# redradman/MujocoPoseLearning

Hardware: AMD Instinct MI355X
Metric: env steps/sec (whole node), humanoid 'stand' task, 1/2/4/8 MI355X (higher is better)
Workload: dtype f64

## Files before the change

mujocoposelearning_amd/csrc/hs_contacts.h:

```cpp
#pragma once
#include "hs_lanes.h"
#include "hs_scratch.h"

namespace hs {
namespace {

template <typename T>
struct Con {
  T pos[3], n[3], t1[3], dist;
};

template <typename T>
__device__ __forceinline__ bool plane_sphere(const T* pp, const T* pn, const T* c, T r, Con<T>& o) {
  T d[3] = {c[0] - pp[0], c[1] - pp[1], c[2] - pp[2]};
  T cd = dot3(d, pn);
  if (cd > r) return false;
  o.dist = cd - r;
  for (int k = 0; k < 3; k++) { o.n[k] = pn[k]; o.pos[k] = c[k] - pn[k] * (o.dist * T(0.5) + r); o.t1[k] = 0; }
  return true;
}
template <typename T>
__device__ __forceinline__ bool sphere_sphere(const T* p1, T r1, const T* p2, T r2, Con<T>& o) {
  T d[3] = {p2[0] - p1[0], p2[1] - p1[1], p2[2] - p1[2]};
  T len = sqrt(dot3(d, d));
  T dist = len - r1 - r2;
  if (dist > 0) return false;
  o.dist = dist;
  if (len < T(1e-15)) { o.n[0] = 1; o.n[1] = 0; o.n[2] = 0; }
  else { T i = recip(len); for (int k = 0; k < 3; k++) o.n[k] = d[k] * i; }
  for (int k = 0; k < 3; k++) { o.pos[k] = p1[k] + o.n[k] * (r1 + dist * T(0.5)); o.t1[k] = 0; }
  return true;
}
template <typename T>
__device__ __forceinline__ void make_frame(Con<T>& c) {
  normalize3(c.n);
  if (sqrt(dot3(c.t1, c.t1)) < T(0.5)) {
    if (fabs(c.n[1]) < T(0.5)) { c.t1[0] = 0; c.t1[1] = 1; c.t1[2] = 0; }
    else { c.t1[0] = 0; c.t1[1] = 0; c.t1[2] = 1; }
  }
  T d = dot3(c.n, c.t1);
  for (int k = 0; k < 3; k++) c.t1[k] -= c.n[k] * d;
  normalize3(c.t1);
}

template <typename T, typename C>
__device__ __forceinline__ int collide_pair(const Scratch<T, C>& s, const int4 info, const T (&sz)[4], Con<T>& c0,
                                           Con<T>& c1) {
  const int g1 = info.x, g2 = info.y, fn = info.z;
  const T* p1 = s.u.k.gpos[g1];
  const T* p2 = s.u.k.gpos[g2];
  const T* a1 = s.u.k.gax[g1];
  const T* a2 = s.u.k.gax[g2];
  const T r1 = sz[0], h1 = sz[1], r2 = sz[2], h2 = sz[3];
  int n = 0;
  if (fn >= PAIR_SPHERE_SPHERE) {
    const T d[3] = {p1[0] - p2[0], p1[1] - p2[1], p1[2] - p2[2]};
    const T R = r1 + h1 + r2 + h2;
    if (dot3(d, d) > R * R) return 0;
  }
  if (fn == PAIR_PLANE_SPHERE) {
    n = plane_sphere(p1, a1, p2, r2, c0) ? 1 : 0;
  } else if (fn == PAIR_PLANE_CAPSULE) {
    T e[3];
    for (int k = 0; k < 3; k++) e[k] = p2[k] + h2 * a2[k];
    Con<T> t;
    if (plane_sphere(p1, a1, e, r2, t)) { for (int k = 0; k < 3; k++) t.t1[k] = a2[k]; c0 = t; n = 1; }
    for (int k = 0; k < 3; k++) e[k] = p2[k] - h2 * a2[k];
    if (plane_sphere(p1, a1, e, r2, t)) {
      for (int k = 0; k < 3; k++) t.t1[k] = a2[k];
      if (n == 0) c0 = t; else c1 = t;
      n++;
    }
  } else if (fn == PAIR_SPHERE_SPHERE) {
    n = sphere_sphere(p1, r1, p2, r2, c0) ? 1 : 0;
  } else if (fn == PAIR_SPHERE_CAPSULE) {
    T d[3] = {p1[0] - p2[0], p1[1] - p2[1], p1[2] - p2[2]};
    T x = dot3(a2, d);
    x = x > h2 ? h2 : (x < -h2 ? -h2 : x);
    T v[3] = {p2[0] + x * a2[0], p2[1] + x * a2[1], p2[2] + x * a2[2]};
    n = sphere_sphere(p1, r1, v, r2, c0) ? 1 : 0;
  } else {
    T ax1[3] = {a1[0] * h1, a1[1] * h1, a1[2] * h1}, ax2[3] = {a2[0] * h2, a2[1] * h2, a2[2] * h2};
    T dif[3] = {p1[0] - p2[0], p1[1] - p2[1], p1[2] - p2[2]};
    T ma = dot3(ax1, ax1), mb = -dot3(ax1, ax2), mc = dot3(ax2, ax2), u = -dot3(ax1, dif), v = dot3(ax2, dif);
    T det = ma * mc - mb * mb;
    T v1[3], v2[3];
    if (fabs(det) >= T(1e-15)) {
      T x1 = (mc * u - mb * v) / det, x2 = (ma * v - mb * u) / det;
      if (x1 > 1) { x1 = 1; x2 = (v - mb) / mc; }
      else if (x1 < -1) { x1 = -1; x2 = (v + mb) / mc; }
      if (x2 > 1) { x2 = 1; x1 = (u - mb) / ma; x1 = x1 > 1 ? 1 : (x1 < -1 ? -1 : x1); }
      else if (x2 < -1) { x2 = -1; x1 = (u + mb) / ma; x1 = x1 > 1 ? 1 : (x1 < -1 ? -1 : x1); }
      for (int k = 0; k < 3; k++) { v1[k] = p1[k] + x1 * ax1[k]; v2[k] = p2[k] + x2 * ax2[k]; }
      n = sphere_sphere(v1, r1, v2, r2, c0) ? 1 : 0;
    } else {
      for (int side = 1; side >= -1; side -= 2) {
        T x2 = (v - side * mb) / mc;
        x2 = x2 > 1 ? 1 : (x2 < -1 ? -1 : x2);
        for (int k = 0; k < 3; k++) { v1[k] = p1[k] + side * ax1[k]; v2[k] = p2[k] + x2 * ax2[k]; }
        Con<T> t;
        if (sphere_sphere(v1, r1, v2, r2, t)) { if (n == 0) c0 = t; else c1 = t; n++; }
      }
    }
  }
  if (n > 0) make_frame(c0);
  if (n > 1) make_frame(c1);
  return n;
}

template <typename T, typename C>
__device__ __forceinline__ void store_contact(MPtr<T> m, Scratch<T, C>& s, int slot, const Con<T>& c, int p) {
  if (slot >= C::CON) return;
  for (int k = 0; k < 3; k++) { s.con_pos[slot][k] = c.pos[k]; s.con_n[slot][k] = c.n[k]; s.con_t1[slot][k] = c.t1[k]; }
  s.con_dist[slot] = c.dist;
  s.con_pair[slot] = p;
  const int b1 = m->pair_b1[p], b2 = m->pair_b2[p];
  s.con_bb[slot] = (uint32_t)b1 | (uint32_t)b2 << 8 | (uint32_t)m->pair_dim[p] << 16;
  s.con_m1[slot] = b1 ? m->body_chainmask[b1] : 0u;
  s.con_m2[slot] = m->body_chainmask[b2];
  s.con_mu[slot] = m->pair_mu[p];
}

template <typename T>
__device__ __forceinline__ T impedance(CPtr<T> si, T pos, T margin) {
  T s0 = fmin(T(0.9999), fmax(T(0.0001), si[0])), s1 = fmin(T(0.9999), fmax(T(0.0001), si[1]));
  if (s0 == s1 || si[2] <= T(1e-15)) return T(0.5) * (s0 + s1);
  T x = (pos - margin) * si[5];
  if (x < 0) x = -x;
  if (x >= 1 || x <= 0) return x >= 1 ? s1 : s0;
  const T p = si[4];
  T y = x;
  if (p != T(1)) {
    const bool lo = x <= si[3];
    const T base = lo ? x : 1 - x;
    T pw = base * base;
    if (p != T(2)) pw = pow(base, p);
    y = lo ? pw * si[6] : 1 - pw * si[7];
  }
  return s0 + y * (s1 - s0);
}

template <typename T>
__device__ __forceinline__ uint32_t chain_mask(MPtr<T> m, int sl, int nb) {
  return (sl > 0 && sl < nb) ? m->body_chainmask[sl] : 0u;
}
template <int NV, typename T, typename C>
__device__ __forceinline__ void map_vx(Scratch<T, C>& s, int sl, int nb, uint32_t ch) {
  if (sl < nb) {
    T v[6] = {0, 0, 0, 0, 0, 0};
    for_bits<T>(ch, [&](int j) { ValsX<T, 6> r; r.x = s.vx[j]; for (int k = 0; k < 6; k++) r.v[k] = s.cdof[j][k]; return r; },
                [&](int, const ValsX<T, 6>& r) {
#pragma unroll
                  for (int k = 0; k < 6; k++) v[k] = fma(r.v[k], r.x, v[k]);
                });
    for (int k = 0; k < 6; k++) s.u.n.bvel[sl][k] = v[k];
  }
  WSYNC();
#pragma unroll
  for (int cs = 0; cs < C::CON; cs += HL) {
    const int c = cs + sl;
    if (c < s.ncon) {
      const uint32_t bb = s.con_bb[c];
      const int b1 = bb & 0xff, b2 = (bb >> 8) & 0xff;
      T r[3] = {s.con_pos[c][0] - s.com[0], s.con_pos[c][1] - s.com[1], s.con_pos[c][2] - s.com[2]};
      T w[3], v1[3], v2[3];
      cross3(s.u.n.bvel[b2], r, w);
      for (int k = 0; k < 3; k++) v2[k] = s.u.n.bvel[b2][3 + k] + w[k];
      cross3(s.u.n.bvel[b1], r, w);
      for (int k = 0; k < 3; k++) v1[k] = s.u.n.bvel[b1][3 + k] + w[k];
      T dv[3] = {v2[0] - v1[0], v2[1] - v1[1], v2[2] - v1[2]};
      T t2[3];
      cross3(s.con_n[c], s.con_t1[c], t2);
      s.con_v[c][0] = dot3(s.con_n[c], dv);
      s.con_v[c][1] = dot3(s.con_t1[c], dv);
      s.con_v[c][2] = dot3(t2, dv);
    }
  }
  WSYNC();
}

template <typename T, typename C>
__device__ __forceinline__ T row_Jx(MPtr<T> m, const Scratch<T, C>& s, int desc, T coef) {
  int kind = rk_kind(desc), j = rk_id(desc);
  if (kind <= RK_JHI) return coef * s.vx[j];
  if (kind <= RK_THI) {
    T v = 0;
    for (int w = 0; w < m->ten_nwrap[j]; w++) v += m->ten_wrapcoef[j][w] * s.vx[m->ten_wrapdof[j][w]];
    return coef * v;
  }
  int comp = kind == RK_CN ? 1 : 1 + ((kind - RK_P0) >> 1);
  return s.con_v[j][0] + coef * s.con_v[j][comp];
}

template <typename T, typename C>
__device__ __forceinline__ void row_u(MPtr<T> m, const Scratch<T, C>& s, int kind, int c, T* u) {
  if (kind == RK_CN) { for (int k = 0; k < 3; k++) u[k] = s.con_n[c][k]; return; }
  int sub = kind - RK_P0;
  T mu = s.con_mu[c];
  T sg = (sub & 1) ? -mu : mu;
  T t[3];
  if (sub >> 1) cross3(s.con_n[c], s.con_t1[c], t);
  else { t[0] = s.con_t1[c][0]; t[1] = s.con_t1[c][1]; t[2] = s.con_t1[c][2]; }
  for (int k = 0; k < 3; k++) u[k] = s.con_n[c][k] + sg * t[k];
}

template <typename T, typename C>
__device__ __forceinline__ void contact_aggregates(MPtr<T> m, Scratch<T, C>& s, int sl) {
  const bool up = threadIdx.x >= HL;
#pragma unroll
  for (int cs = 0; cs < C::CON; cs += HL) {
    const int c = cs + sl;
    bool act = false;
    if (c < s.ncon) {
      int adr = s.con_adr[c];
      int nr = (s.con_bb[c] >> 16) == 1 ? 1 : 4;
      T U[6] = {0, 0, 0, 0, 0, 0}, F[3] = {0, 0, 0};
      const bool pyr = nr == 4;
      T f4[4], D4[4], nn[3], t1[3], t2[3];
#pragma unroll
      for (int q = 0; q < 4; q++) {
        const bool on = q == 0 || pyr;
        f4[q] = on ? s.row_f[adr + q] : T(0);
        D4[q] = on ? s.row_D[adr + q] : T(0);
      }
      for (int k = 0; k < 3; k++) { nn[k] = s.con_n[c][k]; t1[k] = s.con_t1[c][k]; }
      const T mu = s.con_mu[c];
      cross3(nn, t1, t2);
#pragma unroll
      for (int q = 0; q < 4; q++) {
        const T f = f4[q];
        if (f != T(0)) {
          T u[3];
          if (!pyr) {
            for (int k = 0; k < 3; k++) u[k] = nn[k];
          } else {
            const T sg = (q & 1) ? -mu : mu;
            for (int k = 0; k < 3; k++) u[k] = nn[k] + sg * ((q >> 1) ? t2[k] : t1[k]);
          }
          const T D = D4[q];
          U[0] += D * u[0] * u[0]; U[1] += D * u[1] * u[1]; U[2] += D * u[2] * u[2];
          U[3] += D * u[0] * u[1]; U[4] += D * u[0] * u[2]; U[5] += D * u[1] * u[2];
          for (int k = 0; k < 3; k++) F[k] += f * u[k];
        }
      }
      for (int k = 0; k < 6; k++) s.con_U[c][k] = U[k];
      for (int k = 0; k < 3; k++) s.con_F[c][k] = F[k];
      act = F[0] != T(0) || F[1] != T(0) || F[2] != T(0) || U[0] != T(0) || U[1] != T(0) || U[2] != T(0);
    }
    const uint32_t mk = hballot(act, up);
    if (sl == 0) s.con_act[cs / HL] = mk;
  }
  WSYNC();
}
template <typename C, typename F>
__device__ __forceinline__ void for_active_contacts(const uint32_t* act, F&& f) {
#pragma unroll
  for (int w = 0; w < (C::CON + HL - 1) / HL; w++)
    for (uint32_t mk = act[w]; mk; mk &= mk - 1u) f(w * HL + __builtin_ctz(mk));
}

template <typename T, typename C, typename LD, typename F>
__device__ __forceinline__ void for_active_contacts_ld(const uint32_t* act, LD&& ld, F&& f) {
#pragma unroll
  for (int w = 0; w < (C::CON + HL - 1) / HL; w++)
    for_bits<T, true>(
        act[w], [&](int j) { return ld(w * HL + j); }, [&](int j, const auto& v) { f(w * HL + j, v); });
}

template <typename T, typename C>
__device__ __forceinline__ T jtf_lane(MPtr<T> m, const Scratch<T, C>& s, int sl, const T* cd) {
  T acc = 0;
  struct CV { uint32_t m1, m2; T p[3], f[3]; };
  for_active_contacts_ld<T, C>(s.con_act, [&](int c) {
    CV v;
    v.m1 = s.con_m1[c]; v.m2 = s.con_m2[c];
    for (int k = 0; k < 3; k++) { v.p[k] = s.con_pos[c][k]; v.f[k] = s.con_F[c][k]; }
    return v;
  }, [&](int, const CV& v) {
    const int in2 = bit(v.m2, sl), in1 = bit(v.m1, sl);
    if (in1 != in2) {
      T r[3] = {v.p[0] - s.com[0], v.p[1] - s.com[1], v.p[2] - s.com[2]};
      T w[3];
      cross3(cd, r, w);
      T jp[3] = {cd[3] + w[0], cd[4] + w[1], cd[5] + w[2]};
      T x = dot3(jp, v.f);
      acc += in2 ? x : -x;
    }
  });
  if (sl < MAXDOF) {
    int lr = s.lim_row[sl];
    int lo = (lr & 0xff) - 1, hi = (lr >> 8) - 1;
    if (lo >= 0) acc += s.row_f[lo];
    if (hi >= 0) acc -= s.row_f[hi];
  }
  for (int r = s.njl; r < s.nlim; r++) {
    int id = rk_id(s.row_kid[r]);
    T f = rk_kind(s.row_kid[r]) == RK_TLO ? s.row_f[r] : -s.row_f[r];
    for (int w = 0; w < m->ten_nwrap[id]; w++)
      if (m->ten_wrapdof[id][w] == sl) acc += f * m->ten_wrapcoef[id][w];
  }
  return acc;
}

}
}
```

mujocoposelearning_amd/csrc/hs_scratch.h:

```cpp
#pragma once
#include <cstdint>

#include "hs_lanes.h"
#include "hs_model.h"

namespace hs {
namespace {

enum RowKind { RK_JLO = 0, RK_JHI = 1, RK_TLO = 2, RK_THI = 3, RK_CN = 4, RK_P0 = 5 };
__device__ __forceinline__ int rk_kind(int kid) { return kid >> 16; }
__device__ __forceinline__ int rk_id(int kid) { return kid & 0xffff; }

template <typename T, typename C>
struct Scratch {
  T qpos[MAXQ];
  T qvel[MAXDOF];
  T ctrl[MAXU];
  alignas(16) T vx[MAXDOF];
  T com[4];
  T cinert[MAXBODY][10];
  T cdof[MAXDOF][6];
  T cvel[MAXBODY][6];
  T con_pos[C::CON][3];
  T con_n[C::CON][3];
  T con_t1[C::CON][3];
  T con_dist[C::CON];
  T con_v[C::CON][3];
  T con_U[C::CON][6];
  T con_F[C::CON][3];
  int con_pair[C::CON];
  int con_adr[C::CON];
  uint32_t con_bb[C::CON];
  uint32_t con_m1[C::CON];
  uint32_t con_m2[C::CON];
  T con_mu[C::CON];
  uint32_t con_act[(C::CON + HL - 1) / HL];
  uint16_t lim_row[MAXDOF];
  uint32_t dense_mask[C::RPL];
  int row_kid[C::EFC];
  T row_D[C::EFC];
  T row_f[C::EFC];
  int ncon, nefc, nlim, njl;
  int niter;
  struct Kin { T xpos[MAXBODY][3]; T xmat[MAXBODY][9]; T xquat[MAXBODY][4]; T xanchor[MAXJNT][3];
               T xaxis[MAXJNT][3]; T gpos[MAXGEOM][3]; T gax[MAXGEOM][3]; };
  union {
    Kin k;
    struct { T crb[MAXBODY][10]; T buf[MAXDOF][6]; } c;
    struct { T cdofdot[MAXDOF][6]; T cfrc[MAXBODY][6]; T csub[MAXBODY][6]; } r;
    struct { T bvel[MAXBODY][6];
             alignas(16) T cb[MAXDOF][2];
             T cfrc[MAXBODY][6], linv[MAXBODY][3], mv[MAXBODY][3]; } n;
    struct { alignas(16) float x[sizeof(T) == 8 ? 512 : 4]; alignas(16) float h[sizeof(T) == 8 ? 256 : 4]; } pol;
  } u;
};

constexpr int PGS_LA = 3;
template <typename T>
constexpr int pgs_cache_rows() { return sizeof(T) == 4 ? 40 : 48; }
template <typename T>
struct alignas(4 * sizeof(T)) PgsRow {
  T b, R, ar, ai;
  T g[4];
};
template <typename T, typename C>
struct PgsCache {
  static constexpr int NC = pgs_cache_rows<T>();
  T u[NC][MAXDOF];
  PgsRow<T> row[C::EFC];
};

}
}
```

mujocoposelearning_amd/csrc/hs_stepper.h:

```cpp
#pragma once
#include "hs_contacts.h"
#include "hs_dense.h"
#include "hs_lanes.h"
#include "hs_phase_clock.h"
#include "hs_scratch.h"

namespace hs {
namespace {

template <typename T, int NV, typename C>
struct Stepper {
  PhaseClock clk;
  MPtr<T> m;
  Scratch<T, C>& s;
  int sl, nb;
  bool up;
  T cd[6];
  T Mr[NV];
  T fsmooth;
  T fcon;
  T qacc;
  T qfa;
  T damp;
  int niter;
  T* dbg = nullptr;

  __device__ Stepper(MPtr<T> mm, Scratch<T, C>& ss, int lane)
      : m(mm), s(ss), sl(lane & (HL - 1)), nb(mm->nbody), up(lane >= HL) {}

  static constexpr bool LDLF = sizeof(T) == 8;
  static constexpr bool LDLE = false;
  __device__ __forceinline__ static KPtr<T> kargs() { return (KPtr<T>)__builtin_amdgcn_kernarg_segment_ptr(); }

  __device__ __forceinline__ void phase_begin() {
    m = opaque(m);
    sl = opaque_v(sl);
  }

  __device__ __forceinline__ void kinematics() {
    phase_begin();
    if (sl == 0) {
      for (int k = 0; k < 3; k++) s.u.k.xpos[0][k] = 0;
      s.u.k.xquat[0][0] = 1; s.u.k.xquat[0][1] = s.u.k.xquat[0][2] = s.u.k.xquat[0][3] = 0;
      for (int k = 0; k < 9; k++) s.u.k.xmat[0][k] = (k % 4 == 0) ? T(1) : T(0);
    }
    const int b = sl;
    const bool isb = b > 0 && b < nb;
    int depth = -1, par = 0, ja = 0, jn = 0, fqa = 0;
    bool isfree = false;
    T pl[3] = {0, 0, 0}, ql[4] = {1, 0, 0, 0};
    T anl[MAXJPB][3], axl[MAXJPB][3];
    if (isb) {
      depth = m->body_depth[b];
      par = m->body_parentid[b];
      ja = m->body_jntadr[b];
      jn = m->body_jntnum[b];
      isfree = jn == 1 && m->jnt_type[ja] == JNT_FREE;
      fqa = m->jnt_qposadr[ja];
      for (int k = 0; k < 3; k++) pl[k] = m->body_pos[b][k];
      for (int k = 0; k < 4; k++) ql[k] = m->body_quat[b][k];
    }
    if (isfree) {
      for (int k = 0; k < 3; k++) pl[k] = s.qpos[fqa + k];
      for (int k = 0; k < 4; k++) ql[k] = s.qpos[fqa + 3 + k];
    }
#pragma unroll
    for (int jj = 0; jj < MAXJPB; jj++) {
      const bool use = isb && !isfree && jj < jn;
      const int j = use ? ja + jj : 0;
      T jp[3], jx[3], ang = 0;
      for (int k = 0; k < 3; k++) { jp[k] = use ? m->jnt_pos[j][k] : T(0); jx[k] = use ? m->jnt_axis[j][k] : T(0); }
      if (use) {
        int qa = m->jnt_qposadr[j];
        ang = s.qpos[qa] - m->qpos0[qa];
      }
      T sn, cs;
      sincos_t(T(0.5) * ang, sn, cs);
      const T jr[4] = {cs, jx[0] * sn, jx[1] * sn, jx[2] * sn};
      T R[9];
      quat2mat(ql, R);
      mv3(R, jx, axl[jj]);
      mv3(R, jp, anl[jj]);
      for (int k = 0; k < 3; k++) anl[jj][k] += pl[k];
      if (use) {
        mulq(ql, jr, ql);
        quat2mat(ql, R);
        T v[3];
        mv3(R, jp, v);
        for (int k = 0; k < 3; k++) pl[k] = anl[jj][k] - v[k];
      }
    }
    WSYNC();
    for (int L = 1; L <= m->nlevel; L++) {
      if (depth == L) {
        T pos[3], q[4];
        if (isfree) {
          for (int k = 0; k < 3; k++) pos[k] = pl[k];
          for (int k = 0; k < 4; k++) q[k] = ql[k];
        } else {
          mv3(s.u.k.xmat[par], pl, pos);
          for (int k = 0; k < 3; k++) pos[k] += s.u.k.xpos[par][k];
          T pq[4] = {s.u.k.xquat[par][0], s.u.k.xquat[par][1], s.u.k.xquat[par][2], s.u.k.xquat[par][3]};
          mulq(pq, ql, q);
        }
        normalize4(q);
        for (int k = 0; k < 4; k++) s.u.k.xquat[b][k] = q[k];
        for (int k = 0; k < 3; k++) s.u.k.xpos[b][k] = pos[k];
        quat2mat(q, s.u.k.xmat[b]);
      }
      WSYNC();
    }
    if (isb) {
      if (isfree) {
        for (int k = 0; k < 3; k++) { s.u.k.xanchor[ja][k] = s.u.k.xpos[b][k]; s.u.k.xaxis[ja][k] = m->jnt_axis[ja][k]; }
      } else {
        const T* Rp = s.u.k.xmat[par];
        const T* xp = s.u.k.xpos[par];
#pragma unroll
        for (int jj = 0; jj < MAXJPB; jj++) {
          if (jj < jn) {
            T an[3], ax[3];
            mv3(Rp, anl[jj], an);
            mv3(Rp, axl[jj], ax);
            for (int k = 0; k < 3; k++) { s.u.k.xanchor[ja + jj][k] = xp[k] + an[k]; s.u.k.xaxis[ja + jj][k] = ax[k]; }
          }
        }
      }
    }
    if (sl < m->ngeom) {
      int g = sl, gb = m->geom_bodyid[g];
      T gp[3] = {m->geom_pos[g][0], m->geom_pos[g][1], m->geom_pos[g][2]};
      T gz[3] = {m->geom_zaxis[g][0], m->geom_zaxis[g][1], m->geom_zaxis[g][2]};
      T w[3];
      mv3(s.u.k.xmat[gb], gp, w);
      for (int k = 0; k < 3; k++) s.u.k.gpos[g][k] = s.u.k.xpos[gb][k] + w[k];
      mv3(s.u.k.xmat[gb], gz, s.u.k.gax[g]);
    }
    T mx = 0, my = 0, mz = 0, xi[3] = {0, 0, 0};
    if (b > 0 && b < nb) {
      T ip[3] = {m->body_ipos[b][0], m->body_ipos[b][1], m->body_ipos[b][2]}, w[3];
      mv3(s.u.k.xmat[b], ip, w);
      for (int k = 0; k < 3; k++) xi[k] = s.u.k.xpos[b][k] + w[k];
      T mb = m->body_mass[b];
      mx = mb * xi[0]; my = mb * xi[1]; mz = mb * xi[2];
    }
    T inv = T(1) / m->total_mass;
    T c0 = hsum(mx) * inv, c1 = hsum(my) * inv, c2 = hsum(mz) * inv;
    if (sl == 0) { s.com[0] = c0; s.com[1] = c1; s.com[2] = c2; }
    if (b > 0 && b < nb) {
      const T* R = s.u.k.xmat[b];
      CPtr<T> I6 = m->body_inert[b];
      T I[9] = {I6[0], I6[3], I6[4], I6[3], I6[1], I6[5], I6[4], I6[5], I6[2]};
      T A[9];
      for (int r = 0; r < 3; r++)
        for (int c = 0; c < 3; c++) A[3 * r + c] = R[3 * r] * I[c] + R[3 * r + 1] * I[3 + c] + R[3 * r + 2] * I[6 + c];
      T Ic[6];
      Ic[0] = A[0] * R[0] + A[1] * R[1] + A[2] * R[2];
      Ic[1] = A[3] * R[3] + A[4] * R[4] + A[5] * R[5];
      Ic[2] = A[6] * R[6] + A[7] * R[7] + A[8] * R[8];
      Ic[3] = A[0] * R[3] + A[1] * R[4] + A[2] * R[5];
      Ic[4] = A[0] * R[6] + A[1] * R[7] + A[2] * R[8];
      Ic[5] = A[3] * R[6] + A[4] * R[7] + A[5] * R[8];
      T d[3] = {xi[0] - c0, xi[1] - c1, xi[2] - c2};
      T mass = m->body_mass[b];
      T* ci = s.cinert[b];
      ci[0] = Ic[0] + mass * (d[1] * d[1] + d[2] * d[2]);
      ci[1] = Ic[1] + mass * (d[0] * d[0] + d[2] * d[2]);
      ci[2] = Ic[2] + mass * (d[0] * d[0] + d[1] * d[1]);
      ci[3] = Ic[3] - mass * d[0] * d[1];
      ci[4] = Ic[4] - mass * d[0] * d[2];
      ci[5] = Ic[5] - mass * d[1] * d[2];
      ci[6] = mass * d[0]; ci[7] = mass * d[1]; ci[8] = mass * d[2]; ci[9] = mass;
    }
    if (sl == 0)
      for (int k = 0; k < 10; k++) s.cinert[0][k] = 0;
    for (int k = 0; k < 6; k++) cd[k] = 0;
    if (sl < NV) {
      int j = m->dof_jntid[sl], db = m->dof_bodyid[sl];
      T off[3] = {c0 - s.u.k.xanchor[j][0], c1 - s.u.k.xanchor[j][1], c2 - s.u.k.xanchor[j][2]};
      T ax[3];
      bool lin = false;
      if (m->jnt_type[j] == JNT_FREE) {
        int k = sl - m->jnt_dofadr[j];
        if (k < 3) {
          lin = true;
          cd[3] = k == 0 ? T(1) : T(0); cd[4] = k == 1 ? T(1) : T(0); cd[5] = k == 2 ? T(1) : T(0);
        } else {
          int c = k - 3;
          ax[0] = s.u.k.xmat[db][c]; ax[1] = s.u.k.xmat[db][3 + c]; ax[2] = s.u.k.xmat[db][6 + c];
        }
      } else {
        ax[0] = s.u.k.xaxis[j][0]; ax[1] = s.u.k.xaxis[j][1]; ax[2] = s.u.k.xaxis[j][2];
      }
      if (!lin) {
        cd[0] = ax[0]; cd[1] = ax[1]; cd[2] = ax[2];
        cross3(ax, off, cd + 3);
      }
      for (int k = 0; k < 6; k++) s.cdof[sl][k] = cd[k];
    }
    WSYNC();
    if (dbg)
      for (int k = sl; k < MAXBODY * 3; k += HL) dbg[k] = s.u.k.xpos[k / 3][k % 3];
  }

  __device__ __forceinline__ int collision() {
    phase_begin();
    int ncon = 0;
    const int npair = m->npair;
    int4 info_n = make_int4(0, 0, 0, 0);
    T sz_n[4] = {0, 0, 0, 0};
    if (sl < npair) {
      info_n = make_int4(m->pair_info[sl][0], m->pair_info[sl][1], m->pair_info[sl][2], m->pair_info[sl][3]);
      for (int k = 0; k < 4; k++) sz_n[k] = m->pair_size[sl][k];
    }
    for (int base = 0; base < npair; base += HL) {
      int p = base + sl;
      Con<T> c0, c1;
      int n = 0;
      const int4 info = info_n;
      T sz[4] = {sz_n[0], sz_n[1], sz_n[2], sz_n[3]};
      if (p + HL < npair) {
        info_n = make_int4(m->pair_info[p + HL][0], m->pair_info[p + HL][1], m->pair_info[p + HL][2],
                           m->pair_info[p + HL][3]);
        for (int k = 0; k < 4; k++) sz_n[k] = m->pair_size[p + HL][k];
      }
      if (p < npair) n = collide_pair(s, info, sz, c0, c1);
      uint32_t m1 = hballot(n >= 1, up), m2 = hballot(n >= 2, up);
      int pre = below(m1, sl) + below(m2, sl);
      if (n >= 1) store_contact(m, s, ncon + pre, c0, p);
      if (n >= 2) store_contact(m, s, ncon + pre + 1, c1, p);
      ncon += __popc(m1) + __popc(m2);
    }
    int overflow = ncon > C::CON;
    if (overflow) ncon = C::CON;
    if (sl == 0) s.ncon = ncon;
    WSYNC();
    return overflow;
  }

  __device__ __forceinline__ void mass_matrix() {
    phase_begin();
    if (sl > 0 && sl < nb) {
      const uint32_t dm = m->body_descmask[sl] & ~1u & ((nb < 32 ? (1u << nb) : 0u) - 1u);
      T a[10] = {0, 0, 0, 0, 0, 0, 0, 0, 0, 0};
      for_bits<T>(dm, [&](int c) { Vals<T, 10> r; for (int k = 0; k < 10; k++) r.v[k] = s.cinert[c][k]; return r; },
                  [&](int, const Vals<T, 10>& r) { for (int k = 0; k < 10; k++) a[k] += r.v[k]; });
      for (int k = 0; k < 10; k++) s.u.c.crb[sl][k] = a[k];
    }
    WSYNC();
    T bf[6] = {0, 0, 0, 0, 0, 0};
    uint32_t anci = 0;
    T arm = 0;
    if (sl < NV) {
      mul_inert(s.u.c.crb[m->dof_bodyid[sl]], cd, bf);
      for (int k = 0; k < 6; k++) s.u.c.buf[sl][k] = bf[k];
      anci = m->dof_ancmask[sl];
      arm = m->dof_armature[sl];
    }
    WSYNC();
    {
      T cb2[2][12];
      auto load = [&](auto jc, T (&dst)[12]) {
        constexpr int j = decltype(jc)::value;
        for (int k = 0; k < 6; k++) { dst[k] = s.cdof[j][k]; dst[6 + k] = s.u.c.buf[j][k]; }
      };
      load(std::integral_constant<int, 0>{}, cb2[0]);
      static_for<0, NV>([&](auto jc) {
        constexpr int j = decltype(jc)::value;
        if constexpr (j + 1 < NV) load(std::integral_constant<int, j + 1>{}, cb2[(j + 1) & 1]);
        SCHED_FENCE();
        const uint32_t ancj = m->dof_ancmask[j];
        const bool rel = (sl < NV) && (bit(anci, j) || bit(ancj, sl));
        const T* cj = cb2[j & 1];
        const T v = (j <= sl) ? dot6(cj, bf) : dot6(cd, cj + 6);
        Mr[j] = rel ? v + ((j == sl) ? arm : T(0)) : T(0);
      });
    }
    WSYNC();
  }

  __device__ __forceinline__ void velocity_forces() {
    phase_begin();
    if (sl < nb) {
      T v[6] = {0, 0, 0, 0, 0, 0};
      if (sl > 0) {
        const uint32_t ch = m->body_chainmask[sl];
        for_bits<T>(ch, [&](int j) { ValsX<T, 6> r; r.x = s.qvel[j]; for (int k = 0; k < 6; k++) r.v[k] = s.cdof[j][k]; return r; },
                    [&](int, const ValsX<T, 6>& r) { for (int k = 0; k < 6; k++) v[k] = fma(r.v[k], r.x, v[k]); });
      }
      for (int k = 0; k < 6; k++) s.cvel[sl][k] = v[k];
    }
    if (sl < NV) {
      const uint32_t dm = m->dof_dotmask[sl];
      T v[6] = {0, 0, 0, 0, 0, 0}, cdd[6];
      for_bits<T>(dm, [&](int j) { ValsX<T, 6> r; r.x = s.qvel[j]; for (int k = 0; k < 6; k++) r.v[k] = s.cdof[j][k]; return r; },
                  [&](int, const ValsX<T, 6>& r) { for (int k = 0; k < 6; k++) v[k] = fma(r.v[k], r.x, v[k]); });
      cross_motion(v, cd, cdd);
      for (int k = 0; k < 6; k++) s.u.r.cdofdot[sl][k] = cdd[k];
    }
    WSYNC();
    if (sl > 0 && sl < nb) {
      const uint32_t ch = m->body_chainmask[sl];
      T a[6] = {0, 0, 0, -m->gravity[0], -m->gravity[1], -m->gravity[2]};
      for_bits<T>(ch, [&](int j) { ValsX<T, 6> r; r.x = s.qvel[j]; for (int k = 0; k < 6; k++) r.v[k] = s.u.r.cdofdot[j][k]; return r; },
                  [&](int, const ValsX<T, 6>& r) { for (int k = 0; k < 6; k++) a[k] = fma(r.v[k], r.x, a[k]); });
      T f[6], t[6], t2[6];
      mul_inert(s.cinert[sl], a, f);
      mul_inert(s.cinert[sl], s.cvel[sl], t);
      cross_force(s.cvel[sl], t, t2);
      for (int k = 0; k < 6; k++) s.u.r.cfrc[sl][k] = f[k] + t2[k];
    }
    WSYNC();
    if (sl > 0 && sl < nb) {
      const uint32_t dm = m->body_descmask[sl] & ~1u & ((nb < 32 ? (1u << nb) : 0u) - 1u);
      T a[6] = {0, 0, 0, 0, 0, 0};
      for_bits<T>(dm, [&](int c) { Vals<T, 6> r; for (int k = 0; k < 6; k++) r.v[k] = s.u.r.cfrc[c][k]; return r; },
                  [&](int, const Vals<T, 6>& r) { for (int k = 0; k < 6; k++) a[k] += r.v[k]; });
      for (int k = 0; k < 6; k++) s.u.r.csub[sl][k] = a[k];
    }
    WSYNC();
    fsmooth = 0;
    qfa = 0;
    if (sl < NV) {
      T bias = dot6(cd, s.u.r.csub[m->dof_bodyid[sl]]);
      int qa = m->dof_qposadr[sl];
      T pas = -m->dof_damping[sl] * s.qvel[sl];
      if (qa >= 0) pas -= m->dof_stiffness[sl] * (s.qpos[qa] - m->dof_springref[sl]);
      int u = m->dof_actuator[sl];
      if (u >= 0) {
        T c = s.ctrl[u];
        if (m->act_ctrllimited[u]) c = fmin(m->act_ctrlrange[u][1], fmax(m->act_ctrlrange[u][0], c));
        qfa = m->act_gear[u] * c;
      }
      fsmooth = pas - bias + qfa;
    }
    WSYNC();
  }

  __device__ __forceinline__ int rows(T (&D)[C::RPL], T (&ar)[C::RPL], int (&rd)[C::RPL], T (&rc)[C::RPL]) {
    phase_begin();
    damp = sl < NV ? m->dof_damping[sl] : T(0);
    int overflow = 0;
    int ncon = s.ncon;
    int nrow = 0;
    {
      bool lo = false, hi = false;
      if (sl < m->njnt && m->jnt_limited[sl]) {
        T q = s.qpos[m->jnt_qposadr[sl]];
        lo = (q - m->jnt_range[sl][0]) < m->jnt_margin[sl];
        hi = (m->jnt_range[sl][1] - q) < m->jnt_margin[sl];
      }
      uint32_t ml = hballot(lo, up), mh = hballot(hi, up);
      int pre = below(ml, sl) + below(mh, sl);
      if (lo) s.row_kid[pre] = (RK_JLO << 16) | sl;
      if (hi) s.row_kid[pre + lo] = (RK_JHI << 16) | sl;
      nrow = __popc(ml) + __popc(mh);
      s.lim_row[sl] = 0;
      if (lo || hi)
        s.lim_row[m->jnt_dofadr[sl]] = (uint16_t)((lo ? pre + 1 : 0) | (hi ? (pre + lo + 1) << 8 : 0));
    }
    const int njl = nrow;
    {
      bool lo = false, hi = false;
      if (sl < m->ntendon && m->ten_limited[sl]) {
        T L = 0;
        for (int w = 0; w < m->ten_nwrap[sl]; w++) L += m->ten_wrapcoef[sl][w] * s.qpos[m->ten_wrapqadr[sl][w]];
        lo = (L - m->ten_range[sl][0]) < m->ten_margin[sl];
        hi = (m->ten_range[sl][1] - L) < m->ten_margin[sl];
      }
      uint32_t ml = hballot(lo, up), mh = hballot(hi, up);
      int pre = nrow + below(ml, sl) + below(mh, sl);
      if (lo) s.row_kid[pre] = (RK_TLO << 16) | sl;
      if (hi) s.row_kid[pre + lo] = (RK_THI << 16) | sl;
      nrow += __popc(ml) + __popc(mh);
    }
    int nlim = nrow;
    {
      int tot = 0;
#pragma unroll
      for (int cs = 0; cs < C::CON; cs += HL) {
        const int c = cs + sl;
        const bool isc = c < ncon;
        const bool pyr = isc && (s.con_bb[c] >> 16) == 3;
        tot += __popc(hballot(isc, up)) + 3 * __popc(hballot(pyr, up));
      }
      if (nrow + tot > C::EFC) {
        overflow = 1;
        int fit = 0, nr = nrow;
        for (int c = 0; c < ncon; c++) {
          int need = (s.con_bb[c] >> 16) == 3 ? 4 : 1;
          if (nr + need > C::EFC) break;
          nr += need;
          fit++;
        }
        ncon = fit;
      }
#pragma unroll
      for (int cs = 0; cs < C::CON; cs += HL) {
        const int c = cs + sl;
        const bool isc = c < ncon;
        const bool pyr = isc && (s.con_bb[c] >> 16) == 3;
        const uint32_t mc = hballot(isc, up), mp = hballot(pyr, up);
        const int pre = nrow + below(mc, sl) + 3 * below(mp, sl);
        if (isc) {
          s.con_adr[c] = pre;
          if (!pyr) s.row_kid[pre] = (RK_CN << 16) | c;
          else for (int q = 0; q < 4; q++) s.row_kid[pre + q] = ((RK_P0 + q) << 16) | c;
        }
        nrow += __popc(mc) + 3 * __popc(mp);
      }
    }
    if (sl == 0) { s.ncon = ncon; s.nefc = nrow; s.nlim = nlim; s.njl = njl; }
    if (sl < NV) s.vx[sl] = s.qvel[sl];
    WSYNC();
    map_vx<NV>(s, sl, nb, chain_mask(m, sl, nb));
#pragma unroll
    for (int q = 0; q < C::RPL; q++) {
      int r = sl + HL * q;
      D[q] = 0;
      ar[q] = 0;
      rd[q] = 0;
      rc[q] = 0;
      bool dense = false;
      if (r < nrow) {
        int kid = s.row_kid[r];
        int kind = rk_kind(kid), id = rk_id(kid);
        T pos, margin, dA, rscale = 1;
        CPtr<T> sr;
        CPtr<T> si;
        if (kind <= RK_JHI) {
          T qv = s.qpos[m->jnt_qposadr[id]];
          pos = kind == RK_JLO ? qv - m->jnt_range[id][0] : m->jnt_range[id][1] - qv;
          margin = m->jnt_margin[id];
          sr = m->jnt_solref[id]; si = m->jnt_solimp[id];
          int dof = m->jnt_dofadr[id];
          dA = m->dof_invweight0[dof];
          rd[q] = (kind << 16) | dof;
          rc[q] = kind == RK_JLO ? T(1) : T(-1);
        } else if (kind <= RK_THI) {
          T L = 0;
          for (int w = 0; w < m->ten_nwrap[id]; w++) L += m->ten_wrapcoef[id][w] * s.qpos[m->ten_wrapqadr[id][w]];
          pos = kind == RK_TLO ? L - m->ten_range[id][0] : m->ten_range[id][1] - L;
          margin = m->ten_margin[id];
          sr = m->ten_solref[id]; si = m->ten_solimp[id];
          dA = m->ten_invweight0[id];
          rd[q] = kid;
          rc[q] = kind == RK_TLO ? T(1) : T(-1);
          dense = true;
        } else {
          int p = s.con_pair[id];
          pos = s.con_dist[id];
          margin = m->pair_margin[p];
          sr = m->pair_solref[p]; si = m->pair_solimp[p];
          const uint32_t bb = s.con_bb[id];
          T tran = m->body_invweight_tran[bb & 0xff] + m->body_invweight_tran[(bb >> 8) & 0xff];
          T mu = s.con_mu[id];
          dA = kind == RK_CN ? tran : tran + mu * mu * tran;
          if (kind != RK_CN) rscale = 2 * mu * mu;
          rd[q] = kid;
          rc[q] = kind == RK_CN ? T(0) : (((kind - RK_P0) & 1) ? -mu : mu);
          dense = s.con_m1[id] != 0u;
        }
        T imp = impedance(si, pos, margin);
        T dmax = fmin(T(0.9999), fmax(T(0.0001), si[1]));
        T K, B;
        if (sr[0] > 0) {
          T tc = fmax(sr[0], 2 * m->timestep), dr = sr[1];
          const T u = recip(dmax * tc), ud = u * recip(dr);
          K = ud * ud;
          B = 2 * u;
        } else {
          const T v = recip(dmax);
          K = -sr[0] * v * v;
          B = -sr[1] * v;
        }
        T R = rscale * fmax(T(1e-15), (1 - imp) * dA * recip(imp));
        D[q] = recip(R);
        s.row_D[r] = D[q];
        ar[q] = -B * row_Jx(m, s, rd[q], rc[q]) - K * imp * (pos - margin);
      }
      uint32_t dm = hballot(dense, up);
      if (sl == 0) s.dense_mask[q] = dm;
    }
    WSYNC();
    return overflow;
  }

  __device__ __forceinline__ void solve(T xws, int maxit, T tol, const T (&D)[C::RPL], const T (&ar)[C::RPL],
                                        const int (&rd)[C::RPL], const T (&rc)[C::RPL]) {
    phase_begin();
    const int nefc = s.nefc;
    T x = sl < NV ? xws : T(0);
    bool vr[C::RPL];
#pragma unroll
    for (int q = 0; q < C::RPL; q++) vr[q] = sl + HL * q < nefc;
    const uint32_t anci = sl < NV ? m->dof_ancmask[sl] : 0u;
    const uint32_t bch = chain_mask(m, sl, nb);
    const T scale = m->newton_scale;
    if (sl < NV) s.vx[sl] = x;
    WSYNC();
    T Mx = matvec_lds(Mr, s.vx);
    map_vx<NV>(s, sl, nb, bch);
    T jar[C::RPL], Js[C::RPL];
#pragma unroll
    for (int q = 0; q < C::RPL; q++) jar[q] = vr[q] ? row_Jx(m, s, rd[q], rc[q]) - ar[q] : T(0);
    HS_STAMP(clk, 6);
    bool done = false;
    int it = 0;
    if (sl == 0) s.niter = maxit;
    for (; it < maxit; it++) {
      m = opaque(m);
      sl = opaque_v(sl);
      bool act[C::RPL];
#pragma unroll
      for (int q = 0; q < C::RPL; q++) {
        act[q] = vr[q] && jar[q] < 0;
        if (vr[q]) s.row_f[sl + HL * q] = act[q] ? -D[q] * jar[q] : T(0);
      }
      WSYNC();
      contact_aggregates(m, s, sl);
      HS_STAMP(clk, 7);
      T jtf = jtf_lane(m, s, sl, cd);
      T g = sl < NV ? Mx - fsmooth - jtf : T(0);
      const T gn2 = hsum(g * g);
      const bool conv = scale * scale * gn2 < tol * tol;
      if (conv && !done && sl == 0) s.niter = it;
      done = done || conv;
      HS_STAMP(clk, 8);
      if (__ballot(!done) == 0) break;
      T H[NV];
      T hdinv = 0, hdiag = 0;
      {
        T aug[6] = {0, 0, 0, 0, 0, 0};
        T dadd = 0;
        struct CU { uint32_t m1, m2; T p[3], U[6]; };
        for_active_contacts_ld<T, C>(s.con_act, [&](int c) {
          CU v;
          v.m1 = s.con_m1[c]; v.m2 = s.con_m2[c];
          for (int k = 0; k < 3; k++) v.p[k] = s.con_pos[c][k];
          for (int k = 0; k < 6; k++) v.U[k] = s.con_U[c][k];
          return v;
        }, [&](int, const CU& v) {
          if (v.m1 != 0u || !bit(v.m2, sl)) return;
          T r[3] = {v.p[0] - s.com[0], v.p[1] - s.com[1], v.p[2] - s.com[2]};
          T w[3];
          cross3(cd, r, w);
          T jp[3] = {cd[3] + w[0], cd[4] + w[1], cd[5] + w[2]};
          const T* U = v.U;
          T z[3] = {U[0] * jp[0] + U[3] * jp[1] + U[4] * jp[2], U[3] * jp[0] + U[1] * jp[1] + U[5] * jp[2],
                    U[4] * jp[0] + U[5] * jp[1] + U[2] * jp[2]};
          T rz[3];
          cross3(r, z, rz);
          for (int k = 0; k < 3; k++) { aug[k] += rz[k]; aug[3 + k] += z[k]; }
        });
        {
          int lr = s.lim_row[sl];
          int lo = (lr & 0xff) - 1, hi = (lr >> 8) - 1;
          if (lo >= 0 && s.row_f[lo] != T(0)) dadd += s.row_D[lo];
          if (hi >= 0 && s.row_f[hi] != T(0)) dadd += s.row_D[hi];
        }
        HS_STAMP(clk, 27);
        constexpr int HESS_G = sizeof(T) == 8 ? 2 : 1;
        if constexpr (HESS_G == 1) {
#pragma unroll
          for (int j = 0; j < NV; j++) {
            T cj[6];
            for (int k = 0; k < 6; k++) cj[k] = s.cdof[j][k];
            H[j] = Mr[j] + (bit(anci, j) ? dot6(cj, aug) : T(0)) + ((j == sl) ? dadd : T(0));
            SCHED_FENCE();
          }
        } else {
          constexpr int NG = (NV + HESS_G - 1) / HESS_G;
          T cbuf[2][HESS_G][6];
          auto load = [&](auto gc, T (&dst)[HESS_G][6]) {
            constexpr int j0 = decltype(gc)::value * HESS_G;
            static_for<0, HESS_G>([&](auto tc) {
              constexpr int t = decltype(tc)::value;
              if constexpr (j0 + t < NV)
                for (int k = 0; k < 6; k++) dst[t][k] = s.cdof[j0 + t][k];
            });
          };
          load(std::integral_constant<int, 0>{}, cbuf[0]);
          static_for<0, NG>([&](auto gc) {
            constexpr int g = decltype(gc)::value, j0 = g * HESS_G;
            if constexpr (g + 1 < NG) load(std::integral_constant<int, g + 1>{}, cbuf[(g + 1) & 1]);
            SCHED_FENCE();
            static_for<0, HESS_G>([&](auto tc) {
              constexpr int t = decltype(tc)::value, j = j0 + t;
              if constexpr (j < NV)
                H[j] = Mr[j] + (bit(anci, j) ? dot6(cbuf[g & 1][t], aug) : T(0)) + ((j == sl) ? dadd : T(0));
            });
          });
        }
        HS_STAMP(clk, 28);
        uint32_t dm[C::RPL];
#pragma unroll
        for (int q = 0; q < C::RPL; q++) dm[q] = s.dense_mask[q] & hballot(act[q], up);
        for (;;) {
          int r = -1;
#pragma unroll
          for (int q = C::RPL - 1; q >= 0; q--)
            if (dm[q]) r = HL * q + __builtin_ctz(dm[q]);
          if (__ballot(r >= 0) == 0) break;
          T jr = 0, Dr = 0;
          if (r >= 0) {
            dm[r / HL] &= dm[r / HL] - 1u;
            if (s.row_f[r] != T(0)) {
              int kid = s.row_kid[r];
              int kind = rk_kind(kid), id = rk_id(kid);
              Dr = s.row_D[r];
              if (kind == RK_TLO || kind == RK_THI) {
                for (int w = 0; w < m->ten_nwrap[id]; w++)
                  if (m->ten_wrapdof[id][w] == sl) jr += m->ten_wrapcoef[id][w];
                if (kind == RK_THI) jr = -jr;
              } else {
                int in2 = bit(s.con_m2[id], sl), in1 = bit(s.con_m1[id], sl);
                if (in1 != in2) {
                  T rr[3] = {s.con_pos[id][0] - s.com[0], s.con_pos[id][1] - s.com[1], s.con_pos[id][2] - s.com[2]};
                  T w[3], u[3];
                  cross3(cd, rr, w);
                  T jp[3] = {cd[3] + w[0], cd[4] + w[1], cd[5] + w[2]};
                  row_u(m, s, kind, id, u);
                  jr = in2 ? dot3(u, jp) : -dot3(u, jp);
                }
              }
            }
          }
          if (sl >= NV) jr = 0;
          T dj = Dr * jr;
          static_for<0, NV>([&](auto jc) {
            constexpr int j = decltype(jc)::value;
            H[j] += dj * bcast<j>(jr);
          });
        }
      }
      HS_STAMP(clk, 9);
      chol_rows<NV, T, LDLF>(H, hdinv, sl, s.u.n.cb, &hdiag);
      HS_STAMP(clk, 15);
      T sdir = -chol_solve<NV, T, LDLF>(H, hdinv, g, sl);
      if (sl >= NV) sdir = 0;
      HS_STAMP(clk, 10);
      if (sl < NV) s.vx[sl] = sdir;
      WSYNC();
      T Ms = matvec_lds(Mr, s.vx);
      T A0 = hsum(sl < NV ? sdir * Ms : T(0));
      T B0 = hsum(sl < NV ? sdir * (Mx - fsmooth) : T(0));
      HS_STAMP(clk, 18);
      map_vx<NV>(s, sl, nb, bch);
      HS_STAMP(clk, 19);
#pragma unroll
      for (int q = 0; q < C::RPL; q++) Js[q] = vr[q] ? row_Jx(m, s, rd[q], rc[q]) : T(0);
      HS_STAMP(clk, 16);
      bool same1 = true;
#pragma unroll
      for (int q = 0; q < C::RPL; q++) same1 = same1 && (!vr[q] || ((jar[q] + Js[q] < 0) == act[q]));
      bool lsdone = done || (hballot(!same1, up) == 0);
      T alpha = 1, lo = 0, hi = T(1e30);
      T d0 = 0;
      {
        T c = 0;
#pragma unroll
        for (int q = 0; q < C::RPL; q++) c += act[q] ? D[q] * jar[q] * Js[q] : T(0);
        d0 = B0 + hsum(c);
      }
      const T ltol = (sizeof(T) == 8 ? T(1e-10) : T(1e-5)) * fabs(d0);
      for (int ls = 0; ls < 30; ls++) {
        if (__ballot(!lsdone) == 0) break;
        T c1 = 0, c2 = 0;
#pragma unroll
        for (int q = 0; q < C::RPL; q++) {
          T jq = jar[q] + alpha * Js[q];
          bool a = vr[q] && jq < 0;
          c1 += a ? D[q] * jq * Js[q] : T(0);
          c2 += a ? D[q] * Js[q] * Js[q] : T(0);
        }
        T d1 = B0 + alpha * A0 + hsum(c1);
        T d2 = A0 + hsum(c2);
        if (!lsdone) {
          if (fabs(d1) <= ltol) {
            lsdone = true;
          } else {
            if (d1 < 0) lo = alpha; else hi = alpha;
            T an = d2 > 0 ? alpha - d1 * recip(d2) : T(-1);
            if (!(an > lo && an < hi)) an = hi < T(1e29) ? T(0.5) * (lo + hi) : T(2) * alpha;
            if (hi - lo <= (sizeof(T) == 8 ? T(1e-14) : T(1e-6)) * hi) lsdone = true;
            else alpha = an;
          }
        }
      }
      HS_STAMP(clk, 11);
      if (!done) {
        x += alpha * sdir;
        Mx += alpha * Ms;
        bool changed = false;
#pragma unroll
        for (int q = 0; q < C::RPL; q++) {
          T nj = jar[q] + alpha * Js[q];
          changed = changed || (vr[q] && ((nj < 0) != act[q]));
          jar[q] = nj;
        }
        if (hballot(changed, up) == 0 && fabs(alpha - T(1)) < T(1e-3)) {
          done = true;
          if (sl == 0) s.niter = it + 1;
        }
      }
      if (__ballot(!done) == 0) { it++; break; }
    }
    WSYNC();
    niter = s.niter;
#pragma unroll
    for (int q = 0; q < C::RPL; q++)
      if (vr[q]) s.row_f[sl + HL * q] = jar[q] < 0 ? -D[q] * jar[q] : T(0);
    WSYNC();
    contact_aggregates(m, s, sl);
    fcon = sl < NV ? jtf_lane(m, s, sl, cd) : T(0);
    qacc = x;
    WSYNC();
    HS_STAMP(clk, 12);
  }

  __device__ __forceinline__ T row_J_lane(int r) {
    if (sl >= NV) return T(0);
    const int kid = s.row_kid[r];
    const int kind = rk_kind(kid), id = rk_id(kid);
    if (kind <= RK_JHI) return m->jnt_dofadr[id] == sl ? (kind == RK_JLO ? T(1) : T(-1)) : T(0);
    if (kind <= RK_THI) {
      T v = 0;
      for (int w = 0; w < m->ten_nwrap[id]; w++)
        if (m->ten_wrapdof[id][w] == sl) v += m->ten_wrapcoef[id][w];
      return kind == RK_TLO ? v : -v;
    }
    const int in2 = bit(s.con_m2[id], sl), in1 = bit(s.con_m1[id], sl);
    if (in1 == in2) return T(0);
    T rr[3] = {s.con_pos[id][0] - s.com[0], s.con_pos[id][1] - s.com[1], s.con_pos[id][2] - s.com[2]};
    T w[3], u[3];
    cross3(cd, rr, w);
    T jp[3] = {cd[3] + w[0], cd[4] + w[1], cd[5] + w[2]};
    row_u(m, s, kind, id, u);
    const T v = dot3(u, jp);
    return in2 ? v : -v;
  }

  __device__ __forceinline__ void solve_pgs(T xws, int maxit, const T (&D)[C::RPL], const T (&ar)[C::RPL],
                                            const int (&rd)[C::RPL], const T (&rc)[C::RPL], PgsCache<T, C>& pc) {
    phase_begin();
    const int nefc = s.nefc;
    const uint32_t bch = chain_mask(m, sl, nb);
    const T fs = sl < NV ? fsmooth : T(0);
    constexpr int NC = PgsCache<T, C>::NC;
    constexpr int LA = PGS_LA;
    bool vr[C::RPL];
#pragma unroll
    for (int q = 0; q < C::RPL; q++) vr[q] = sl + HL * q < nefc;
    T L[NV];
#pragma unroll
    for (int j = 0; j < NV; j++) L[j] = Mr[j];
    T dinv = 0;
    chol_rows<NV>(L, dinv, sl, s.u.n.cb);
    if (sl < NV) s.vx[sl] = xws;
    WSYNC();
    map_vx<NV>(s, sl, nb, bch);
    T wc = 0;
#pragma unroll
    for (int q = 0; q < C::RPL; q++) {
      const int r = sl + HL * q;
      if (vr[q]) {
        const T jar = row_Jx(m, s, rd[q], rc[q]) - ar[q];
        const T f = jar < 0 ? -D[q] * jar : T(0);
        const T R = recip(D[q]);
        s.row_f[r] = f;
        pc.row[r].b = -ar[q];
        pc.row[r].R = R;
        wc += f * (T(0.5) * R * f - ar[q]);
      }
    }
    WSYNC();
    int maxr = nefc;
    maxr = max(maxr, __shfl_xor(maxr, HL));
    constexpr int G = sizeof(T) == 8 ? 4 : 8;
    const int ncache = maxr < NC ? maxr : NC;
    for (int r0 = 0; r0 < ncache; r0 += G) {
      T y[G];
      static_for<0, G>([&](auto gc) {
        constexpr int g = decltype(gc)::value;
        y[g] = r0 + g < nefc ? row_J_lane(r0 + g) : T(0);
      });
      chol_fwd_multi<NV, G>(L, dinv, y, sl);
      static_for<0, G>([&](auto gc) {
        constexpr int g = decltype(gc)::value;
        if (r0 + g < NC) pc.u[r0 + g][sl] = sl < NV ? y[g] : T(0);
      });
    }
    WSYNC();
    auto urow = [&](int r) -> T {
      if (r < NC) return pc.u[r][sl];
      T y = chol_fwd<NV>(L, dinv, r < nefc ? row_J_lane(r) : T(0), sl);
      return sl < NV ? y : T(0);
    };
    {
      T uw[LA + 1];
#pragma unroll
      for (int j = 0; j < LA; j++) uw[j] = 0;
      for (int r = 0; r < maxr; r++) {
        uw[LA] = urow(r);
        const T a = hsum(uw[LA] * uw[LA]);
        T gr[LA];
#pragma unroll
        for (int j = 1; j <= LA; j++) gr[j - 1] = hsum(uw[LA] * uw[LA - j]);
        if (r < nefc && sl == 0) {
          const T arr = a + pc.row[r].R;
          pc.row[r].ar = arr;
          pc.row[r].ai = recip(arr < T(1e-15) ? T(1e-15) : arr);
#pragma unroll
          for (int j = 0; j < LA; j++) pc.row[r].g[j] = gr[j];
        }
#pragma unroll
        for (int j = 0; j < LA; j++) uw[j] = uw[j + 1];
      }
    }
    WSYNC();
    contact_aggregates(m, s, sl);
    T z, y0;
    {
      T y2[2] = {fs, fs + (sl < NV ? jtf_lane(m, s, sl, cd) : T(0))};
      chol_fwd_multi<NV, 2>(L, dinv, y2, sl);
      y0 = sl < NV ? y2[0] : T(0);
      z = sl < NV ? y2[1] : T(0);
    }
    if (hsum(wc + T(0.5) * (z * z - y0 * y0)) > T(0)) {
#pragma unroll
      for (int q = 0; q < C::RPL; q++)
        if (vr[q]) s.row_f[sl + HL * q] = 0;
      z = y0;
    }
    WSYNC();
    const T scale = m->newton_scale, tol = m->pgs_tol;
    bool done = false;
    int it = 0;
    for (int sweep = 0; sweep < maxit; sweep++) {
      m = opaque(m);
      sl = opaque_v(sl);
      T improvement = 0;
      auto sweep_rows = [&](auto fastc) {
        constexpr bool FAST = decltype(fastc)::value;
        auto uget = [&](int r) -> T {
          if constexpr (FAST) return pc.u[r][sl];
          else return urow(r);
        };
        constexpr int RING = LA + 1;
        static_assert(RING % 2 == 0, "P/F double buffer alternates with the row parity");
        T U[RING], S[RING], Dl[RING];
#pragma unroll
        for (int i = 0; i < RING; i++) {
          U[i] = (i < LA && i < maxr) ? uget(i) : T(0);
          S[i] = i < LA ? hsum(U[i] * z) : T(0);
          Dl[i] = 0;
        }
        PgsRow<T> P[2];
        T F[2];
        P[0] = pc.row[0];
        F[0] = nefc > 0 ? s.row_f[0] : T(0);
        T unext = LA < maxr ? uget(LA) : T(0);
        for (int r0 = 0; r0 < maxr; r0 += RING) {
          static_for<0, RING>([&](auto ic) {
            constexpr int i = decltype(ic)::value;
            constexpr int prev = (i + RING - 1) % RING;
            constexpr int cur = i & 1, nxt = cur ^ 1;
            const int r = r0 + i;
            {
              const int rn = r + 1 < C::EFC ? r + 1 : C::EFC - 1;
              P[nxt] = pc.row[rn];
              const T fl = s.row_f[rn];
              F[nxt] = r + 1 < nefc ? fl : T(0);
            }
            const T un = unext;
            unext = r + LA + 1 < maxr ? uget(r + LA + 1) : T(0);
            z = fma(Dl[prev], U[prev], z);
            const T Sn = hsum(un * z);
            const bool row = r < nefc;
            const bool live = row && !done;
            const PgsRow<T>& pr = P[cur];
            const T fr = F[cur];
            T dot = S[i];
            static_for<1, LA + 1>([&](auto jc) {
              constexpr int j = decltype(jc)::value;
              dot = fma(Dl[(i + RING - j) % RING], pr.g[j - 1], dot);
            });
            const T res = dot + (pr.b + pr.R * fr);
            T nf = fr - res * pr.ai;
            nf = nf < T(0) ? T(0) : nf;
            const T delta = live ? nf - fr : T(0);
            const T di = delta * res + T(0.5) * pr.ar * delta * delta;
            improvement -= row ? di : T(0);
            if (live && sl == 0) s.row_f[r] = nf;
            U[prev] = un;
            S[prev] = Sn;
            Dl[i] = delta;
          });
        }
        z = fma(Dl[RING - 1], U[RING - 1], z);
      };
      if (maxr <= NC) sweep_rows(std::true_type{});
      else sweep_rows(std::false_type{});
      if (!done) it++;
      done = done || (improvement * scale < tol);
      if (__ballot(!done) == 0) break;
      if ((sweep & (sizeof(T) == 8 ? 31 : 7)) == (sizeof(T) == 8 ? 31 : 7)) {
        WSYNC();
        contact_aggregates(m, s, sl);
        const T zz = chol_fwd<NV>(L, dinv, fs + (sl < NV ? jtf_lane(m, s, sl, cd) : T(0)), sl);
        z = sl < NV ? zz : T(0);
      }
    }
    niter = it;
    WSYNC();
    contact_aggregates(m, s, sl);
    fcon = sl < NV ? jtf_lane(m, s, sl, cd) : T(0);
    const T qa = chol_solve<NV>(L, dinv, fs + fcon, sl);
    qacc = sl < NV ? qa : T(0);
    WSYNC();
  }

  __device__ __forceinline__ void post_constraint() {
    phase_begin();
    const int b = sl;
    T cf[6] = {0, 0, 0, 0, 0, 0}, mv[3] = {0, 0, 0};
    if (b > 0 && b < nb) {
      for (int c = 0; c < s.ncon; c++) {
        const uint32_t bb = s.con_bb[c];
        const int b1 = bb & 0xff, b2 = (bb >> 8) & 0xff;
        if (b != b1 && b != b2) continue;
        const T sg = b == b2 ? T(1) : T(-1);
        T r[3] = {s.con_pos[c][0] - s.com[0], s.con_pos[c][1] - s.com[1], s.con_pos[c][2] - s.com[2]}, t[3];
        cross3(r, s.con_F[c], t);
        for (int k = 0; k < 3; k++) { cf[k] += sg * t[k]; cf[3 + k] += sg * s.con_F[c][k]; }
      }
      const T* ci = s.cinert[b];
      const T* cv = s.cvel[b];
      T w[3];
      cross3(cv, ci + 6, w);
      for (int k = 0; k < 3; k++) mv[k] = ci[9] * cv[3 + k] + w[k];
    }
    if (b < nb) {
      for (int k = 0; k < 6; k++) s.u.n.cfrc[b][k] = cf[k];
      for (int k = 0; k < 3; k++) s.u.n.mv[b][k] = mv[k];
    }
    WSYNC();
    if (b < nb) {
      const uint32_t dm = b == 0 ? ((1u << nb) - 2u) : m->body_descmask[b];
      T a[3] = {0, 0, 0}, ms = 0;
      for (int c = 1; c < nb; c++)
        if (bit(dm, c)) {
          for (int k = 0; k < 3; k++) a[k] += s.u.n.mv[c][k];
          ms += s.cinert[c][9];
        }
      const T inv = T(1) / (ms > T(1e-15) ? ms : T(1e-15));
      for (int k = 0; k < 3; k++) s.u.n.linv[b][k] = a[k] * inv;
    }
    WSYNC();
  }

  __device__ __forceinline__ void euler(T& time) {
    phase_begin();
    T h = m->timestep;
    T He[NV];
#pragma unroll
    for (int j = 0; j < NV; j++) He[j] = Mr[j] + ((j == sl) ? h * damp : T(0));
    HS_STAMP(clk, 20);
    T edinv = 0, ediag = 0;
    chol_rows<NV, T, LDLE>(He, edinv, sl, s.u.n.cb, &ediag);
    HS_STAMP(clk, 21);
    T a = chol_solve<NV, T, LDLE>(He, edinv, fsmooth + fcon, sl);
    HS_STAMP(clk, 17);
    if (sl < NV) s.qvel[sl] += h * a;
    WSYNC();
    if (sl < m->njnt) {
      int qa = m->jnt_qposadr[sl], da = m->jnt_dofadr[sl];
      if (m->jnt_type[sl] == JNT_FREE) {
        for (int k = 0; k < 3; k++) s.qpos[qa + k] += h * s.qvel[da + k];
        T w[3] = {s.qvel[da + 3], s.qvel[da + 4], s.qvel[da + 5]};
        T ang = h * normalize3(w);
        T sn, cs;
        sincos_t(T(0.5) * ang, sn, cs);
        T qr[4] = {cs, w[0] * sn, w[1] * sn, w[2] * sn};
        T q[4] = {s.qpos[qa + 3], s.qpos[qa + 4], s.qpos[qa + 5], s.qpos[qa + 6]};
        normalize4(q);
        mulq(q, qr, q);
        for (int k = 0; k < 4; k++) s.qpos[qa + 3 + k] = q[k];
      } else {
        s.qpos[qa] += h * s.qvel[da];
      }
    }
    time += h;
    WSYNC();
  }
};

}
}
```

Baseline: 6.641 million.

## Prefilter collision pairs with cheap bounds and compact near-pair list

```diff
diff --git a/mujocoposelearning_amd/csrc/hs_contacts.h b/mujocoposelearning_amd/csrc/hs_contacts.h
--- a/mujocoposelearning_amd/csrc/hs_contacts.h
+++ b/mujocoposelearning_amd/csrc/hs_contacts.h
@@ -41,6 +41,19 @@
   T d = dot3(c.n, c.t1);
   for (int k = 0; k < 3; k++) c.t1[k] -= c.n[k] * d;
   normalize3(c.t1);
+}
+
+template <typename T>
+__device__ __forceinline__ bool near_bodies(const T* p1, const T* p2, T R) {
+  const T d[3] = {p1[0] - p2[0], p1[1] - p2[1], p1[2] - p2[2]};
+  return !(dot3(d, d) > R * R);
+}
+template <typename T>
+__device__ __forceinline__ bool near_plane(const T* pp, const T* pn, const T* c, T rb) {
+  const T d[3] = {c[0] - pp[0], c[1] - pp[1], c[2] - pp[2]};
+  const T mag = fabs(c[0]) + fabs(c[1]) + fabs(c[2]) + fabs(pp[0]) + fabs(pp[1]) + fabs(pp[2]) + rb;
+  const T margin = (sizeof(T) == 8 ? T(0x1p-42) : T(0x1p-13)) * (T(1) + mag);
+  return !(dot3(d, pn) > rb + margin);
 }
 
 template <typename T, typename C>
diff --git a/mujocoposelearning_amd/csrc/hs_scratch.h b/mujocoposelearning_amd/csrc/hs_scratch.h
--- a/mujocoposelearning_amd/csrc/hs_scratch.h
+++ b/mujocoposelearning_amd/csrc/hs_scratch.h
@@ -38,6 +38,8 @@
   uint16_t lim_row[MAXDOF];
   uint32_t dense_mask[C::RPL];
   int row_kid[C::EFC];
+  static_assert(sizeof(int) * C::EFC >= MAXPAIR, "the near-pair list fits row_kid");
+  __device__ __forceinline__ uint8_t* near_pairs() { return reinterpret_cast<uint8_t*>(row_kid); }
   T row_D[C::EFC];
   T row_f[C::EFC];
   int ncon, nefc, nlim, njl;
diff --git a/mujocoposelearning_amd/csrc/hs_stepper.h b/mujocoposelearning_amd/csrc/hs_stepper.h
--- a/mujocoposelearning_amd/csrc/hs_stepper.h
+++ b/mujocoposelearning_amd/csrc/hs_stepper.h
@@ -203,28 +203,84 @@
       for (int k = sl; k < MAXBODY * 3; k += HL) dbg[k] = s.u.k.xpos[k / 3][k % 3];
   }
 
+  static constexpr bool COMPACT = sizeof(T) == 8;
   __device__ __forceinline__ int collision() {
     phase_begin();
     int ncon = 0;
     const int npair = m->npair;
+    const uint8_t* near = nullptr;
+    int cnt = npair;
+    int nmax = npair;
+    if constexpr (COMPACT) {
+      constexpr int NPASS = MAXPAIR / HL;
+      static_assert(MAXPAIR % HL == 0 && MAXPAIR <= 256, "whole passes; pair indices fit the byte list");
+      uint8_t* const list = s.near_pairs();
+      int nlo = 0, nhi = 0;
+      int g1[NPASS], g2[NPASS], fn[NPASS];
+      T sz[NPASS][4];
+      T p1[NPASS][3], p2[NPASS][3];
+#pragma unroll
+      for (int ps = 0; ps < NPASS; ps++) {
+        g1[ps] = g2[ps] = fn[ps] = 0;
+        for (int k = 0; k < 4; k++) sz[ps][k] = 0;
+        if (ps * HL < npair) {
+          const int p = ps * HL + sl < npair ? ps * HL + sl : 0;
+          g1[ps] = m->pair_info[p][0]; g2[ps] = m->pair_info[p][1]; fn[ps] = m->pair_info[p][2];
+          for (int k = 0; k < 4; k++) sz[ps][k] = m->pair_size[p][k];
+        }
+      }
+#pragma unroll
+      for (int ps = 0; ps < NPASS; ps++)
+        for (int k = 0; k < 3; k++) {
+          p1[ps][k] = p2[ps][k] = 0;
+          if (ps * HL < npair) { p1[ps][k] = s.u.k.gpos[g1[ps]][k]; p2[ps][k] = s.u.k.gpos[g2[ps]][k]; }
+        }
+      cnt = 0;
+#pragma unroll
+      for (int ps = 0; ps < NPASS; ps++) {
+        if (ps * HL >= npair) continue;
+        const int p = ps * HL + sl;
+        const T r1 = sz[ps][0], h1 = sz[ps][1], r2 = sz[ps][2], h2 = sz[ps][3];
+        bool keep;
+        if (fn[ps] >= PAIR_SPHERE_SPHERE) keep = near_bodies(p1[ps], p2[ps], r1 + h1 + r2 + h2);
+        else keep = near_plane(p1[ps], s.u.k.gax[g1[ps]], p2[ps], fn[ps] == PAIR_PLANE_CAPSULE ? r2 + h2 : r2);
+        keep = keep && p < npair;
+        const uint64_t bm = __ballot(keep);
+        const uint32_t bl = (uint32_t)bm, bh = (uint32_t)(bm >> 32);
+        if (keep) list[cnt + below(up ? bh : bl, sl)] = (uint8_t)p;
+        cnt += __popc(up ? bh : bl);
+        nlo += __popc(bl);
+        nhi += __popc(bh);
+      }
+      WSYNC();
+      near = list;
+      nmax = nlo > nhi ? nlo : nhi;
+    }
+    auto pair_at = [&](int i) -> int {
+      if constexpr (COMPACT) return near[i];
+      else return i;
+    };
+    int p_n = 0;
     int4 info_n = make_int4(0, 0, 0, 0);
     T sz_n[4] = {0, 0, 0, 0};
-    if (sl < npair) {
-      info_n = make_int4(m->pair_info[sl][0], m->pair_info[sl][1], m->pair_info[sl][2], m->pair_info[sl][3]);
-      for (int k = 0; k < 4; k++) sz_n[k] = m->pair_size[sl][k];
-    }
-    for (int base = 0; base < npair; base += HL) {
-      int p = base + sl;
+    if (sl < cnt) {
+      p_n = pair_at(sl);
+      info_n = make_int4(m->pair_info[p_n][0], m->pair_info[p_n][1], m->pair_info[p_n][2], m->pair_info[p_n][3]);
+      for (int k = 0; k < 4; k++) sz_n[k] = m->pair_size[p_n][k];
+    }
+    for (int base = 0; base < nmax; base += HL) {
+      const int i = base + sl;
+      const int p = p_n;
       Con<T> c0, c1;
       int n = 0;
       const int4 info = info_n;
       T sz[4] = {sz_n[0], sz_n[1], sz_n[2], sz_n[3]};
-      if (p + HL < npair) {
-        info_n = make_int4(m->pair_info[p + HL][0], m->pair_info[p + HL][1], m->pair_info[p + HL][2],
-                           m->pair_info[p + HL][3]);
-        for (int k = 0; k < 4; k++) sz_n[k] = m->pair_size[p + HL][k];
-      }
-      if (p < npair) n = collide_pair(s, info, sz, c0, c1);
+      if (i + HL < cnt) {
+        p_n = pair_at(i + HL);
+        info_n = make_int4(m->pair_info[p_n][0], m->pair_info[p_n][1], m->pair_info[p_n][2], m->pair_info[p_n][3]);
+        for (int k = 0; k < 4; k++) sz_n[k] = m->pair_size[p_n][k];
+      }
+      if (i < cnt) n = collide_pair(s, info, sz, c0, c1);
       uint32_t m1 = hballot(n >= 1, up), m2 = hballot(n >= 2, up);
       int pre = below(m1, sl) + below(m2, sl);
       if (n >= 1) store_contact(m, s, ncon + pre, c0, p);
```

Result: no change. 6.683 million, median of 6 (+0.6%).
